# indutny/elliptic

Hardware: NVIDIA H100
Metric: secp256k1 ECDSA verifies/sec (higher is better)
Workload: dtype u32 limbs (integer, exact)

## Files before the change

elliptic_b200/csrc/eb200.cu:

```cuda
#include <cuda_runtime.h>
#include <stdio.h>
#include <string.h>
#include <atomic>
#include <condition_variable>
#include <cstdlib>
#include <mutex>
#include <thread>
#include <type_traits>
#include <vector>
#include "../../include/elliptic_b200.h"
#include "ecdsa_k256_body.cuh"
#include "ecdsa_k256_replay.cuh"
#include "ecdsa_sw_replay.cuh"
#include "ecdsa_k256_sign_fast.cuh"
#include "der_sig.cuh"
#include "ecdsa_sw_sign.cuh"
#include "ecdsa_k256_sign.cuh"
#include "ecdsa_sw_body.cuh"
#include "ed25519_body.cuh"
#include "ed25519_ec.cuh"
#include "sw_runtime.cuh"
#include "kernel_bounds.h"
#include "recovery_param.h"
#include "keyset.h"

using namespace eb;

__global__ void __launch_bounds__(128) k256_gtab_kernel(u32* gtab) {
  size_t t = (size_t)blockIdx.x * blockDim.x + threadIdx.x;
  if (t >= (size_t)GTAB_WINDOWS * GTAB_ENTRIES) return;
  int j = (int)(t / GTAB_ENTRIES), idx = (int)(t % GTAB_ENTRIES);
  gtab_entry(j, idx, gtab + t * 16);
}

__global__ void __launch_bounds__(128) k256_prep_kernel(size_t N, const uint8_t* __restrict__ e,
                                                        const uint8_t* __restrict__ r,
                                                        const uint8_t* __restrict__ s,
                                                        u32* __restrict__ ws, u32* __restrict__ scratch) {
  size_t tid = (size_t)blockIdx.x * blockDim.x + threadIdx.x;
  size_t T = (size_t)gridDim.x * blockDim.x;
  prep_thread(tid, T, N, e, r, s, ws, scratch);
}

__global__ void __launch_bounds__(EB_VERIFY_BLOCK, EB_VERIFY_MINBLOCKS)
k256_verify_kernel(size_t N, const uint8_t* __restrict__ pub, const uint8_t* __restrict__ r,
                   const u32* __restrict__ ws, const u32* __restrict__ gtab,
                   u32* __restrict__ qtab, const uint8_t* __restrict__ pre, uint8_t* __restrict__ status) {
  size_t i = (size_t)blockIdx.x * blockDim.x + threadIdx.x;
  if (i >= N) return;
  if (pre && pre[i]) { status[i] = pre[i]; return; }
  status[i] = verify_item(i, N, pub, r, ws, gtab, qtab);
}

__global__ void __launch_bounds__(128) k256_prep_recover_kernel(size_t N, const uint8_t* __restrict__ e,
                                                                const uint8_t* __restrict__ r,
                                                                const uint8_t* __restrict__ s,
                                                                u32* __restrict__ ws, u32* __restrict__ scratch) {
  size_t tid = (size_t)blockIdx.x * blockDim.x + threadIdx.x;
  size_t T = (size_t)gridDim.x * blockDim.x;
  prep_thread(tid, T, N, e, r, s, ws, scratch, 1);
}
__global__ void __launch_bounds__(EB_VERIFY_BLOCK, EB_VERIFY_MINBLOCKS)
k256_recover_kernel(size_t N, const uint8_t* __restrict__ r, const uint8_t* __restrict__ recid,
                    const u32* __restrict__ ws, const u32* __restrict__ gtab, u32* __restrict__ qtab,
                    uint8_t* __restrict__ out, uint8_t* __restrict__ status) {
  size_t i = (size_t)blockIdx.x * blockDim.x + threadIdx.x;
  if (i >= N) return;
  status[i] = recover_item(i, N, r, recid, ws, gtab, qtab, out);
}

__global__ void __launch_bounds__(128)
k256_sign_nonce_kernel(size_t N, const uint8_t* __restrict__ e, const uint8_t* __restrict__ priv,
                       const u32* __restrict__ gtab, u32* __restrict__ ws, uint8_t* __restrict__ status,
                       const uint8_t* __restrict__ kgiven) {
  size_t i = (size_t)blockIdx.x * blockDim.x + threadIdx.x;
  if (i < N) k256_sign_nonce_item(i, N, e, priv, gtab, ws, status, kgiven);
}
__global__ void __launch_bounds__(128)
k256_sign_finish_kernel(size_t N, const uint8_t* __restrict__ e, const uint8_t* __restrict__ priv, u32 canonical,
                        const u32* __restrict__ ws, u32* __restrict__ scratch, uint8_t* __restrict__ r,
                        uint8_t* __restrict__ s, uint8_t* __restrict__ recid, uint8_t* __restrict__ status) {
  size_t tid = (size_t)blockIdx.x * blockDim.x + threadIdx.x;
  size_t T = (size_t)gridDim.x * blockDim.x;
  k256_sign_finish_thread(tid, T, N, e, priv, canonical, ws, scratch, r, s, recid, status);
}
__global__ void __launch_bounds__(128)
k256_sign_slow_kernel(size_t N, const uint8_t* __restrict__ e, const uint8_t* __restrict__ priv, u32 canonical,
                      const u32* __restrict__ gtab, uint8_t* __restrict__ r, uint8_t* __restrict__ s,
                      uint8_t* __restrict__ recid, uint8_t* __restrict__ status) {
  size_t i = (size_t)blockIdx.x * blockDim.x + threadIdx.x;
  if (i >= N || status[i] != ST_NEEDS_HOST) return;
  status[i] = k256_sign_item(i, e, priv, canonical, gtab, r, s, recid);
}

__global__ void __launch_bounds__(128) k256_replay_tab_kernel(u32* tab) {
  int t = blockIdx.x * blockDim.x + threadIdx.x;
  if (t < 2 * REPLAY_NAF_PTS) rp_tab_entry(t, tab + 16 * t);
}
__global__ void __launch_bounds__(128)
k256_replay_kernel(size_t N, const uint8_t* __restrict__ e, const uint8_t* __restrict__ r, const uint8_t* __restrict__ s,
                   const uint8_t* __restrict__ pub, const u32* __restrict__ tab, uint8_t* __restrict__ status) {
  size_t i = (size_t)blockIdx.x * blockDim.x + threadIdx.x;
  if (i >= N || status[i] != ST_NEEDS_HOST) return;
  status[i] = rp_verify_item(i, e, r, s, pub, tab);
}

__global__ void __launch_bounds__(128)
k256_prep_scalars_kernel(size_t N, const uint8_t* __restrict__ k1, const uint8_t* __restrict__ k2, u32* __restrict__ ws) {
  size_t i = (size_t)blockIdx.x * blockDim.x + threadIdx.x;
  if (i < N) prep_scalars_item(i, N, k1, k2, ws);
}
__global__ void __launch_bounds__(EB_VERIFY_BLOCK, EB_VERIFY_MINBLOCKS)
k256_mul_add_kernel(size_t N, const uint8_t* __restrict__ pts, const u32* __restrict__ ws, const u32* __restrict__ gtab,
                    u32* __restrict__ qtab, uint8_t* __restrict__ out, uint8_t* __restrict__ status) {
  size_t i = (size_t)blockIdx.x * blockDim.x + threadIdx.x;
  if (i >= N) return;
  status[i] = mul_add_item(i, N, pts, ws, gtab, qtab, out);
}
__global__ void __launch_bounds__(128)
k256_mul_add_replay_kernel(size_t N, const uint8_t* __restrict__ k1, const uint8_t* __restrict__ k2,
                           const uint8_t* __restrict__ pts, const u32* __restrict__ tab, uint8_t* __restrict__ out,
                           uint8_t* __restrict__ status) {
  size_t i = (size_t)blockIdx.x * blockDim.x + threadIdx.x;
  if (i >= N || status[i] != ST_NEEDS_HOST) return;
  status[i] = rp_mul_add_item(i, k1, k2, pts, tab, out);
}
__global__ void __launch_bounds__(128)
// ... 398 lines not shown
    for (auto& t : workers_) t.join();
  }
 private:
  void loop() {
    unsigned long long seen = 0;
    for (;;) {
      { std::unique_lock<std::mutex> lk(m_); cv_work_.wait(lk, [&] { return stop_ || gen_ != seen; }); if (stop_) return; seen = gen_; }
      work();
    }
  }
  void work() {
    for (;;) {
      int i = next_.fetch_add(1);
      if (i >= njobs_.load()) break;
      const CopyJob* j = jobs_.load();
      memcpy(j[i].dst, j[i].src, j[i].bytes);
      std::lock_guard<std::mutex> lk(m_);
      if (--pending_ == 0) cv_done_.notify_all();
    }
  }
  std::mutex m_, call_mu_;
  std::condition_variable cv_work_, cv_done_;
  std::vector<std::thread> workers_;
  std::atomic<const CopyJob*> jobs_{nullptr};
  std::atomic<int> njobs_{0}, next_{0};
  int pending_ = 0;
  unsigned long long gen_ = 0;
  bool stop_ = false;
};

enum { EV_START, EV_INPUTS_RESIDENT, EV_KERNELS_DONE, EV_OUTPUTS_HOME, EV_MAIN_BEGIN, EV_MAIN_END, EV_SLOTS };

struct Ctx {
  std::mutex mu;
  bool ready = false;
  int device = -1;
  cudaStream_t stream = nullptr, stream2 = nullptr, copy_stream = nullptr;
  u32* gtab[MAX_CURVES] = {};
  u32* sw_replay_tab[MAX_CURVES] = {};
  u32* replay_tab = nullptr;
  uint8_t* d_in = nullptr; size_t d_in_cap = 0;
  uint8_t* d_ws = nullptr; size_t d_ws_cap = 0;
  uint8_t* d_status = nullptr; size_t d_status_cap = 0;
  cudaEvent_t ev[EV_SLOTS] = {};
  cudaEvent_t ev_in[MAX_CHUNKS] = {}, ev_k0[MAX_CHUNKS] = {}, ev_k1[MAX_CHUNKS] = {}, ev_done[MAX_CHUNKS] = {};
  uint8_t* h_stage[STAGE_SLOTS] = {};
  cudaEvent_t ev_stage[STAGE_SLOTS] = {};
  bool stage_used[STAGE_SLOTS] = {};
  unsigned stage_next = 0;
  CopyPool pool;
  eb200_timing timing = {};
};
Ctx g_ctx[MAX_DEV];
int g_devs[MAX_DEV];
int g_ndev = 0;
std::atomic<unsigned> g_rr{0};
std::mutex g_mu;
thread_local char g_err[256] = "";
thread_local eb200_timing t_timing = {};
thread_local Ctx* t_pending = nullptr;
thread_local unsigned t_pending_launches = 0;

int cuda_fail(cudaError_t e, const char* what) {
  snprintf(g_err, sizeof g_err, "%s: %s", what, cudaGetErrorString(e));
  return (e == cudaErrorNoDevice || e == cudaErrorInsufficientDriver) ? EB200_ERR_NO_DEVICE : EB200_ERR_CUDA;
}
#define CK(call) do { cudaError_t e_ = (call); if (e_ != cudaSuccess) return cuda_fail(e_, #call); } while (0)

struct Launch {
  cudaStream_t st;
  unsigned count = 0;
  int rc = EB200_OK;
  template <class... P, class... A>
  void operator()(void (*kernel)(P...), unsigned grid, unsigned block, A... args) {
    if (rc) return;
    kernel<<<grid, block, 0, st>>>(args...);
    count++;
    cudaError_t e = cudaGetLastError();
    if (e != cudaSuccess) rc = cuda_fail(e, "cudaGetLastError()");
  }
};
unsigned blocks128(size_t threads) { return (unsigned)((threads + 127) / 128); }
unsigned batch_blocks(size_t n, int batch) { return blocks128((n + batch - 1) / batch); }

struct K256Curve {};
struct Ed25519Curve {};
template <class C_> struct SwCurve {
  typedef C_ C;
  typedef SWSign<C, std::conditional_t<std::is_same<C, P384>::value, Sha384W,
                                       std::conditional_t<std::is_same<C, P521>::value, Sha512W, Sha256W>>> SG;
};
template <class T> constexpr bool is_k256 = std::is_same<T, K256Curve>::value;
template <class T> constexpr bool is_ed25519 = std::is_same<T, Ed25519Curve>::value;

template <class F>
int with_curve(int curve, F&& f) {
  switch (curve) {
    case EB200_CURVE_SECP256K1: return f(K256Curve{});
    case EB200_CURVE_ED25519: return f(Ed25519Curve{});
    case EB200_CURVE_P256: return f(SwCurve<P256>{});
    case EB200_CURVE_P384: return f(SwCurve<P384>{});
    case EB200_CURVE_P521: return f(SwCurve<P521>{});
    case EB200_CURVE_P192: return f(SwCurve<P192>{});
    case EB200_CURVE_P224: return f(SwCurve<P224>{});
    default: return EB200_ERR_UNSUPPORTED;
  }
}

[[maybe_unused]] const void* const sw_kernel_order[] = {
    (const void*)sw_decode_pub_kernel<P256>, (const void*)sw_decode_pub_kernel<P384>, (const void*)sw_decode_pub_kernel<P521>,
    (const void*)sw_decode_pub_kernel<P192>, (const void*)sw_decode_pub_kernel<P224>,
    (const void*)sw_keygen_kernel<SwCurve<P256>::SG>, (const void*)sw_keygen_kernel<SwCurve<P384>::SG>,
    (const void*)sw_keygen_kernel<SwCurve<P521>::SG>, (const void*)sw_keygen_kernel<SwCurve<P192>::SG>,
    (const void*)sw_keygen_kernel<SwCurve<P224>::SG>,
    (const void*)sw_mul_g_kernel<P256>, (const void*)sw_mul_g_kernel<P384>, (const void*)sw_mul_g_kernel<P521>,
    (const void*)sw_mul_g_kernel<P192>, (const void*)sw_mul_g_kernel<P224>,
    (const void*)sw_selftest_fe_kernel<P256>, (const void*)sw_selftest_fe_kernel<P384>, (const void*)sw_selftest_fe_kernel<P521>,
    (const void*)sw_selftest_fe_kernel<P192>, (const void*)sw_selftest_fe_kernel<P224>,
};

int grow(uint8_t** p, size_t* cap, size_t need) {
  if (*cap >= need) return EB200_OK;
  if (*p) { cudaFree(*p); *p = nullptr; *cap = 0; }
  CK(cudaMalloc(p, need));
  *cap = need;
  return EB200_OK;
}
size_t align256(size_t x) { return (x + 255) & ~(size_t)255; }

size_t fe_len(int curve) {
  if (curve == EB200_CURVE_P192) return 24;
  return (curve == EB200_CURVE_P384) ? 48 : (curve == EB200_CURVE_P521) ? 72 :
         ((curve >= EB200_CURVE_SECP256K1 && curve <= EB200_CURVE_CURVE25519) || curve == EB200_CURVE_P224) ? 32 : 0;
}
size_t curve_len(int curve) {
  switch (curve) {
    case EB200_CURVE_SECP256K1: case EB200_CURVE_P256: case EB200_CURVE_ED25519: return 32;
    case EB200_CURVE_P384: return 48;
    case EB200_CURVE_P521: return 66;
    case EB200_CURVE_P192: return 24;
    case EB200_CURVE_P224: return 28;
    default: return 0;
  }
}
size_t pub_item_bytes(size_t len, u32 fmt) {
  return fmt == EB200_PUB_XY ? 2 * len : fmt == EB200_PUB_SEC1_65 ? 1 + 2 * len : fmt == EB200_PUB_SEC1_33 ? 1 + len : 0;
}

struct WsLayout { size_t ws, scratch, qtab, xy, pre, total; };
WsLayout ws_layout(int curve, size_t n) {
  size_t prep_words = 0, scratch_words = 0, qtab_words = 0, len = curve_len(curve);
  with_curve(curve, [&](auto cv) {
    typedef decltype(cv) T;
    if constexpr (is_k256<T>) { prep_words = PREP_WORDS; scratch_words = 8; qtab_words = QTAB_WORDS; }
    else if constexpr (is_ed25519<T>) qtab_words = ED_ATAB_WORDS;
    else { typedef SW<typename T::C> W; prep_words = W::PREP_WORDS; scratch_words = W::N; qtab_words = W::QTAB_WORDS; }
    return EB200_OK;
  });
  WsLayout L;
  L.ws = 0;
  L.scratch = align256(L.ws + prep_words * n * 4);
  L.qtab = align256(L.scratch + scratch_words * n * 4);
  L.xy = align256(L.qtab + qtab_words * n * 4);
  L.pre = align256(L.xy + 2 * len * n);
  L.total = align256(L.pre + n);
  return L;
// ... 41 lines not shown
          CK(cudaMemcpyAsync(dsts[j], jobs[j].dst, jobs[j].bytes, cudaMemcpyHostToDevice, st));
          CK(cudaEventRecord(c.ev_stage[slots[j]], st));
          c.stage_used[slots[j]] = true;
        }
        nj = 0;
      }
    }
  }
  if (nj) {
    c.pool.run(jobs, nj);
    for (int j = 0; j < nj; j++) {
      CK(cudaMemcpyAsync(dsts[j], jobs[j].dst, jobs[j].bytes, cudaMemcpyHostToDevice, st));
      CK(cudaEventRecord(c.ev_stage[slots[j]], st));
      c.stage_used[slots[j]] = true;
    }
  }
  return EB200_OK;
}

int ensure_table(Ctx& c, int curve) {
  return with_curve(curve, [&](auto cv) {
    typedef decltype(cv) T;
    if (c.gtab[curve]) return EB200_OK;
    if constexpr (is_k256<T>) {
      size_t entries = (size_t)GTAB_WINDOWS * GTAB_ENTRIES;
      CK(cudaMalloc(&c.gtab[curve], entries * 16 * 4));
      k256_gtab_kernel<<<blocks128(entries), 128, 0, c.stream>>>(c.gtab[curve]);
      CK(cudaGetLastError());
      CK(cudaMalloc(&c.replay_tab, (size_t)REPLAY_TAB_WORDS * 4));
      k256_replay_tab_kernel<<<2, 128, 0, c.stream>>>(c.replay_tab);
    } else if constexpr (is_ed25519<T>) {
      size_t entries = (size_t)ED_GWINDOWS * ED_GENTRIES;
      CK(cudaMalloc(&c.gtab[curve], entries * 24 * 4));
      ed_gtab_kernel<<<blocks128(entries), 128, 0, c.stream>>>(c.gtab[curve]);
    } else {
      typedef typename T::C C;
      typedef SW<C> W;
      size_t entries = (size_t)W::GWINDOWS * W::GENTRIES;
      CK(cudaMalloc(&c.gtab[curve], entries * 2 * W::N * 4));
      sw_gtab_kernel<C><<<blocks128(entries), 128, 0, c.stream>>>(c.gtab[curve]);
      CK(cudaGetLastError());
      CK(cudaMalloc(&c.sw_replay_tab[curve], (size_t)SWReplay<C>::TAB_WORDS * 4));
      sw_replay_tab_kernel<C><<<1, 128, 0, c.stream>>>(c.sw_replay_tab[curve]);
    }
    CK(cudaGetLastError());
    CK(cudaStreamSynchronize(c.stream));
    return EB200_OK;
  });
}

int launch_verify(Ctx& c, int curve, size_t n, const uint8_t* d_e, const uint8_t* d_r, const uint8_t* d_s,
                  const uint8_t* d_pub, u32 pub_fmt, uint8_t* d_status, uint8_t* d_workspace, Launch& L,
                  cudaEvent_t ev_main0, cudaEvent_t ev_main1,
                  const uint8_t* d_der = nullptr, const unsigned long long* d_der_off = nullptr) {
  if (n == 0) return EB200_OK;
  const WsLayout W = ws_layout(curve, n);
  u32* ws = (u32*)(d_workspace + W.ws);
  u32* scratch = (u32*)(d_workspace + W.scratch);
  u32* qtab = (u32*)(d_workspace + W.qtab);
  uint8_t* dxy = d_workspace + W.xy;
  uint8_t* dpre = d_workspace + W.pre;
  const uint8_t* xy = d_pub;
  const uint8_t* pre = nullptr;
  const unsigned nb = blocks128(n);
  const u32* gt = c.gtab[curve];
  return with_curve(curve, [&](auto cv) {
    typedef decltype(cv) T;
    if (pub_fmt != EB200_PUB_XY) {
      if constexpr (is_k256<T>) L(k256_decode_pub_kernel, nb, 128, n, d_pub, pub_fmt, dxy, dpre);
      else if constexpr (is_ed25519<T>) L(ed_ec_decode_pub_kernel, nb, 128, n, d_pub, pub_fmt, dxy, dpre);
      else L(sw_decode_pub_kernel<typename T::C>, nb, 128, n, d_pub, pub_fmt, dxy, dpre);
      xy = dxy; pre = dpre;
    }
    if (d_der) {
      L(der_decode_kernel, nb, 128, n, (u32)curve_len(curve), d_der, d_der_off, (uint8_t*)d_r, (uint8_t*)d_s, dpre,
        (int)(pre != nullptr));
      pre = dpre;
    }
    if constexpr (is_ed25519<T>) {
      CK(cudaEventRecord(ev_main0, L.st));
      L(ed_ec_verify_kernel, nb, 128, n, d_e, d_r, d_s, xy, pre, gt, qtab, d_status);
      CK(cudaEventRecord(ev_main1, L.st));
    } else if constexpr (is_k256<T>) {
      L(k256_prep_kernel, batch_blocks(n, PREP_BATCH), 128, n, d_e, d_r, d_s, ws, scratch);
      CK(cudaEventRecord(ev_main0, L.st));
      L(k256_verify_kernel, (unsigned)((n + EB_VERIFY_BLOCK - 1) / EB_VERIFY_BLOCK), EB_VERIFY_BLOCK, n, xy, d_r, ws, gt,
        qtab, pre, d_status);
      CK(cudaEventRecord(ev_main1, L.st));
      L(k256_replay_kernel, nb, 128, n, d_e, d_r, d_s, xy, c.replay_tab, d_status);
    } else {
      typedef typename T::C C;
      L(sw_prep_kernel<C>, batch_blocks(n, SW<C>::BATCH), 128, n, d_e, d_r, d_s, ws, scratch);
      CK(cudaEventRecord(ev_main0, L.st));
      L(sw_verify_kernel<C>, nb, 128, n, xy, d_r, ws, gt, qtab, pre, d_status);
      CK(cudaEventRecord(ev_main1, L.st));
      L(sw_replay_kernel<C>, nb, 128, n, d_e, d_r, d_s, xy, c.sw_replay_tab[curve], d_status);
    }
    return L.rc;
  });
}

bool curve_ok(int curve) { return curve_len(curve) != 0; }
bool fmt_ok(u32 fmt) { return fmt == EB200_PUB_XY || fmt == EB200_PUB_SEC1_65 || fmt == EB200_PUB_SEC1_33; }

int ctx_create(Ctx& c, int device) {
  CK(cudaSetDevice(device));
  c.device = device;
  CK(cudaStreamCreateWithFlags(&c.stream, cudaStreamNonBlocking));
  CK(cudaStreamCreateWithFlags(&c.copy_stream, cudaStreamNonBlocking));
  CK(cudaStreamCreateWithFlags(&c.stream2, cudaStreamNonBlocking));
  for (int i = 0; i < EV_SLOTS; i++) CK(cudaEventCreate(&c.ev[i]));
  for (int i = 0; i < MAX_CHUNKS; i++) {
    CK(cudaEventCreate(&c.ev_in[i]));
    CK(cudaEventCreate(&c.ev_k0[i]));
    CK(cudaEventCreate(&c.ev_k1[i]));
    CK(cudaEventCreate(&c.ev_done[i]));
  }
  c.ready = true;
  return EB200_OK;
}
void ctx_destroy(Ctx& c) {
  if (c.device < 0) return;
  cudaSetDevice(c.device);
  if (c.stream) cudaStreamSynchronize(c.stream);
  for (int k = 0; k < MAX_CURVES; k++) if (c.gtab[k]) { cudaFree(c.gtab[k]); c.gtab[k] = nullptr; }
  for (int k = 0; k < MAX_CURVES; k++) if (c.sw_replay_tab[k]) { cudaFree(c.sw_replay_tab[k]); c.sw_replay_tab[k] = nullptr; }
  if (c.replay_tab) { cudaFree(c.replay_tab); c.replay_tab = nullptr; }
  if (c.d_in) { cudaMemset(c.d_in, 0, c.d_in_cap); cudaFree(c.d_in); } c.d_in = nullptr; c.d_in_cap = 0;
  if (c.d_ws) { cudaMemset(c.d_ws, 0, c.d_ws_cap); cudaFree(c.d_ws); } c.d_ws = nullptr; c.d_ws_cap = 0;
  cudaFree(c.d_status); c.d_status = nullptr; c.d_status_cap = 0;
  for (int i = 0; i < EV_SLOTS; i++) if (c.ev[i]) { cudaEventDestroy(c.ev[i]); c.ev[i] = nullptr; }
  for (int i = 0; i < MAX_CHUNKS; i++) {
    if (c.ev_in[i]) { cudaEventDestroy(c.ev_in[i]); c.ev_in[i] = nullptr; }
    if (c.ev_k0[i]) { cudaEventDestroy(c.ev_k0[i]); c.ev_k0[i] = nullptr; }
    if (c.ev_k1[i]) { cudaEventDestroy(c.ev_k1[i]); c.ev_k1[i] = nullptr; }
    if (c.ev_done[i]) { cudaEventDestroy(c.ev_done[i]); c.ev_done[i] = nullptr; }
  }
  for (int s = 0; s < STAGE_SLOTS; s++) {
    if (c.h_stage[s]) { memset(c.h_stage[s], 0, STAGE_BYTES); cudaFreeHost(c.h_stage[s]); c.h_stage[s] = nullptr; }
    if (c.ev_stage[s]) { cudaEventDestroy(c.ev_stage[s]); c.ev_stage[s] = nullptr; }
    c.stage_used[s] = false;
  }
  if (c.stream) { cudaStreamDestroy(c.stream); c.stream = nullptr; }
  if (c.copy_stream) { cudaStreamDestroy(c.copy_stream); c.copy_stream = nullptr; }
  if (c.stream2) { cudaStreamDestroy(c.stream2); c.stream2 = nullptr; }
  c.ready = false;
  c.device = -1;
}

Ctx* ctx_of(const void* dptr) {
  cudaPointerAttributes a;
  if (cudaPointerGetAttributes(&a, dptr) != cudaSuccess) { cudaGetLastError(); return nullptr; }
  if (a.type != cudaMemoryTypeDevice && a.type != cudaMemoryTypeManaged) return nullptr;
  if (a.device < 0 || a.device >= MAX_DEV || !g_ctx[a.device].ready) return nullptr;
  return &g_ctx[a.device];
}

void merge_timing(eb200_timing& a, const eb200_timing& b) {
  if (b.h2d_ms > a.h2d_ms) a.h2d_ms = b.h2d_ms;
  if (b.kernel_ms > a.kernel_ms) a.kernel_ms = b.kernel_ms;
  if (b.d2h_ms > a.d2h_ms) a.d2h_ms = b.d2h_ms;
  if (b.main_kernel_ms > a.main_kernel_ms) a.main_kernel_ms = b.main_kernel_ms;
  a.launches += b.launches;
}

template <class F>
int run_sharded_on(const int* devs, int nd, size_t n, F&& fn) {
// ... 1004 lines not shown
namespace {
std::mutex g_ks_mu;
std::vector<eb200_keyset*> g_keysets;

void keyset_free_device(eb200_keyset* ks) {
  for (int i = 0; i < ks->ndev; i++) {
    KeysetDev& d = ks->dev[ks->devs[i]];
    if (cudaSetDevice(ks->devs[i]) != cudaSuccess) { cudaGetLastError(); continue; }
    cudaFree(d.xy); cudaFree(d.kst); cudaFree(d.tab);
    d = KeysetDev{};
  }
  ks->ndev = 0;
  ks->live = false;
}

int keyset_build_on(Ctx& c, eb200_keyset* ks, const uint8_t* pub, uint8_t* key_status) {
  const int curve = ks->curve;
  const size_t m = ks->m, len = curve_len(curve), pb = pub_item_bytes(len, ks->fmt);
  const int windows = keyset_windows(curve, (int)ks->W);
  int rc = ensure_table(c, curve);
  if (rc) return rc;
  KeysetDev& d = ks->dev[c.device];
  d.W = (int)ks->W;
  CK(cudaMalloc(&d.xy, 2 * len * m));
  CK(cudaMalloc(&d.kst, m));
  CK(cudaMalloc(&d.tab, keyset_key_bytes(curve, (int)ks->W) * m));
  if ((rc = grow(&c.d_in, &c.d_in_cap, align256(m * pb) + m))) return rc;
  if ((rc = grow(&c.d_ws, &c.d_ws_cap, m * windows * 3 * keyset_geom(curve).limbs * 4))) return rc;
  uint8_t *d_pub = c.d_in, *d_pre = c.d_in + align256(m * pb);
  return run_single(c, {{d_pub, pub, m * pb}},
    [&](Launch& L) {
      const uint8_t* pre = nullptr;
      if (ks->fmt == EB200_PUB_XY) CK(cudaMemcpyAsync(d.xy, d_pub, 2 * len * m, cudaMemcpyDeviceToDevice, L.st));
      else {
        pre = d_pre;
        int rc2 = with_curve(curve, [&](auto cv) {
          typedef decltype(cv) T;
          if constexpr (is_k256<T>) L(k256_decode_pub_kernel, blocks128(m), 128, m, d_pub, ks->fmt, d.xy, d_pre);
          else if constexpr (is_ed25519<T>) return EB200_ERR_UNSUPPORTED;
          else L(sw_decode_pub_kernel<typename T::C>, blocks128(m), 128, m, d_pub, ks->fmt, d.xy, d_pre);
          return L.rc;
        });
        if (rc2) return rc2;
      }
      cudaError_t err = keyset_build_launch(curve, m, d, pre, (u32*)c.d_ws, L.st, &L.count);
      return err == cudaSuccess ? EB200_OK : cuda_fail(err, "keyset_build_launch");
    },
    {{key_status, d.kst, m}}, {}, true);
}

int verify_keyed_on(Ctx& c, const eb200_keyset* ks, size_t n, const uint8_t* e, const uint8_t* r, const uint8_t* s,
                    const u32* key_idx, uint8_t* status) {
  const int curve = ks->curve;
  const KeysetDev& d = ks->dev[c.device];
  if (!d.tab) return EB200_ERR_NOT_INIT;
  int rc = ensure_table(c, curve);
  if (rc) return rc;
  const size_t len = curve_len(curve);
  const ChunkPlan P = make_plan(n);
  const size_t idx_bytes = align256(n * 4);
  if ((rc = grow(&c.d_in, &c.d_in_cap, idx_bytes + align256(n * 3 * len) + 1024))) return rc;
  const WsLayout W = ws_layout(curve, P.max_m);
  const size_t ws_slot = W.qtab;
  if ((rc = grow(&c.d_ws, &c.d_ws_cap, (P.chunks > 1 ? 2 : 1) * ws_slot))) return rc;
  if ((rc = grow(&c.d_status, &c.d_status_cap, n))) return rc;
  u32* d_idx = (u32*)c.d_in;
  uint8_t *d_e = c.d_in + idx_bytes, *d_r = d_e + n * len, *d_s = d_r + n * len;
  return run_chunked(c, P,
    [&](size_t lo, size_t m, Seg* seg) {
      seg[0] = {d_e + lo * len, e + lo * len, m * len};
      seg[1] = {d_r + lo * len, r + lo * len, m * len};
      seg[2] = {d_s + lo * len, s + lo * len, m * len};
      seg[3] = {d_idx + lo, key_idx + lo, m * 4};
      return 4;
    },
    [&](size_t lo, size_t m, Launch& L, int slot, int k) {
      u32* ws = (u32*)(c.d_ws + (size_t)slot * ws_slot + W.ws);
      u32* scratch = (u32*)(c.d_ws + (size_t)slot * ws_slot + W.scratch);
      const u32* replay = nullptr;
      int rc2 = with_curve(curve, [&](auto cv) {
        typedef decltype(cv) T;
        if constexpr (is_ed25519<T>) return EB200_ERR_UNSUPPORTED;
        else if constexpr (is_k256<T>) {
          L(k256_prep_kernel, batch_blocks(m, PREP_BATCH), 128, m, d_e + lo * len, d_r + lo * len, d_s + lo * len, ws, scratch);
          replay = c.replay_tab;
        } else {
          typedef typename T::C C;
          L(sw_prep_kernel<C>, batch_blocks(m, SW<C>::BATCH), 128, m, d_e + lo * len, d_r + lo * len, d_s + lo * len, ws, scratch);
          replay = c.sw_replay_tab[curve];
        }
        return L.rc;
      });
      if (rc2) return rc2;
      const KeyedVerifyArgs a{d_e + lo * len, d_r + lo * len, d_s + lo * len, d_idx + lo, c.d_status + lo, ws, c.gtab[curve], replay};
      cudaError_t err = keyset_verify_launch(curve, m, d, a, L.st, c.ev_k0[k], c.ev_k1[k], &L.count);
      return err == cudaSuccess ? EB200_OK : cuda_fail(err, "keyset_verify_launch");
    },
    [&](size_t lo, size_t m, Seg* seg) {
      seg[0] = {status + lo, c.d_status + lo, m};
      return 1;
    });
}
}

static void keysets_release_all() {
  std::lock_guard<std::mutex> lk(g_ks_mu);
  for (eb200_keyset* ks : g_keysets) keyset_free_device(ks);
  g_keysets.clear();
}

extern "C" {

int eb200_keyset_create(int curve, size_t m, const uint8_t* pub, uint32_t pub_fmt, uint32_t table_bits,
                        uint8_t* key_status, eb200_keyset** out) {
  if (out) *out = nullptr;
  if (!out || !pub || !key_status || m == 0 || m > 0xffffffffull || !fmt_ok(pub_fmt)) return EB200_ERR_ARG;
  if (table_bits && (table_bits < EB200_KEYSET_MIN_BITS || table_bits > EB200_KEYSET_MAX_BITS)) return EB200_ERR_ARG;
  if (!keyset_geom(curve).limbs) return EB200_ERR_UNSUPPORTED;
  if (!table_bits && !(table_bits = keyset_choose_bits(curve, m, EB200_KEYSET_DEFAULT_BUDGET))) {
    snprintf(g_err, sizeof g_err, "the tables of %zu keys do not fit the default budget at any width: pass table_bits", m);
    return EB200_ERR_ARG;
  }
  int devs[MAX_DEV], nd;
  { std::lock_guard<std::mutex> lk(g_mu); nd = g_ndev; for (int i = 0; i < nd; i++) devs[i] = g_devs[i]; }
  if (nd == 0) return EB200_ERR_NOT_INIT;
  eb200_keyset* ks = new eb200_keyset;
  ks->curve = curve; ks->m = m; ks->W = table_bits; ks->fmt = pub_fmt;
  ks->device_bytes = 2 * curve_len(curve) * m + m + keyset_key_bytes(curve, (int)table_bits) * m;
  t_pending = nullptr;
  eb200_timing tm = {};
  int rc = EB200_OK;
  for (int i = 0; i < nd && !rc; i++) {
    Ctx& c = g_ctx[devs[i]];
    std::lock_guard<std::mutex> lk(c.mu);
    cudaError_t e = cudaSetDevice(c.device);
    if (e != cudaSuccess) { rc = cuda_fail(e, "cudaSetDevice"); break; }
    ks->devs[ks->ndev++] = c.device;
    c.timing = eb200_timing{};
    rc = keyset_build_on(c, ks, pub, key_status);
    merge_timing(tm, c.timing);
  }
  t_timing = tm;
  if (rc) {
    keyset_free_device(ks);
    delete ks;
    return rc;
  }
  ks->live = true;
  { std::lock_guard<std::mutex> lk(g_ks_mu); g_keysets.push_back(ks); }
  *out = ks;
  return EB200_OK;
}

int eb200_keyset_info(const eb200_keyset* ks, int* curve, size_t* m, uint32_t* table_bits, size_t* device_bytes) {
  if (!ks) return EB200_ERR_ARG;
  if (curve) *curve = ks->curve;
  if (m) *m = ks->m;
  if (table_bits) *table_bits = ks->W;
  if (device_bytes) *device_bytes = ks->device_bytes;
  return EB200_OK;
}

int eb200_keyset_destroy(eb200_keyset* ks) {
  if (!ks) return EB200_OK;
  {
    std::lock_guard<std::mutex> lk(g_ks_mu);
    for (size_t i = 0; i < g_keysets.size(); i++)
// ... 22 lines not shown
```

elliptic_b200/csrc/ecdsa_k256_body.cuh:

```cuda
#pragma once
#include "ge_k256.cuh"
#include "sc_k256.cuh"
#ifndef EB_K256_FQ
#define EB_K256_FQ 0
#endif
#include "gq_k256.cuh"

namespace eb {

enum : uint8_t {
  ST_FALSE = 0, ST_TRUE = 1, ST_THROW_INVALID_POINT = 2, ST_THROW_NOT_VALIDATED = 3,
  ST_NEEDS_HOST = 4, ST_THROW_ASSERT = 5, ST_THROW_POINT_FORMAT = 6, ST_INFINITY = 7, ST_THROW_SECOND_KEY = 8, ST_THROW_SIG_FORMAT = 9,
  ST_THROW_NO_RECOVERY = 11,
};

constexpr int PREP_WORDS = 19;
constexpr u32 FL_INVALID = 1, FL_NEGG = 2, FL_NEG1 = 4, FL_NEG2 = 8, FL_NOG = 16;
constexpr int PREP_BATCH = 16;
constexpr int QTAB_ENTRIES = 8;
#if EB_K256_FQ
constexpr int QTAB_WORDS = QTABQ_WORDS;
#else
constexpr int QTAB_WORDS = QTAB_ENTRIES * 24;
#endif
// ... 8 lines not shown
struct madd_out { ge_jac r; fe h; };

#if defined(__CUDACC__)
#define EB_FN __host__ __device__ __noinline__
#else
#define EB_FN
#endif

EB_FN ge_jac jac_dbl(ge_jac p) { return jac_dbl_inl(p); }
EB_FN ge_jac jac_madd(ge_jac a, ge_aff p) { return jac_madd_inl(a, p); }

EB_HD madd_out jac_madd_h(const ge_jac& a, const ge_aff& p) {
  madd_out o;
  fe z2 = fe_sqr(a.z);
  fe u2 = fe_mul(p.x, z2);
  fe s2 = fe_mul(fe_mul(p.y, z2), a.z);
  fe h = fe_sub(a.x, u2);
  fe rr = fe_sub(a.y, s2);
  fe h2 = fe_sqr(h);
  fe h3 = fe_mul(h2, h);
  fe v = fe_mul(a.x, h2);
  o.r.x = fe_sub(fe_sub(fe_add(fe_sqr(rr), h3), v), v);
  o.r.y = fe_sub(fe_mul(rr, fe_sub(v, o.r.x)), fe_mul(a.y, h3));
  o.r.z = fe_mul(a.z, h);
  o.h = h;
  return o;
}

EB_HD fe fe_beta() {
  fe b;
  const u32 v[8] = {0x719501eeu, 0xc1396c28u, 0x12f58995u, 0x9cf04975u, 0xac3434e9u, 0x6e64479eu, 0x657c0710u, 0x7ae96a2bu};
  for (int i = 0; i < 8; i++) b.v[i] = v[i];
  return b;
}

EB_HD ge_aff k256_G() {
  ge_aff g;
  const u32 x[8] = {0x16f81798u, 0x59f2815bu, 0x2dce28d9u, 0x029bfcdbu, 0xce870b07u, 0x55a06295u, 0xf9dcbbacu, 0x79be667eu};
  const u32 y[8] = {0xfb10d4b8u, 0x9c47d08fu, 0xa6855419u, 0xfd17b448u, 0x0e1108a8u, 0x5da4fbfcu, 0x26a3c465u, 0x483ada77u};
  for (int i = 0; i < 8; i++) { g.x.v[i] = x[i]; g.y.v[i] = y[i]; }
  return g;
}

EB_HD void gtab_entry(int j, int idx, u32* out16) {
  ge_jac b = jac_from_aff(k256_G());
  for (int k = 0; k < GTAB_W * j; k++) b = jac_dbl(b);
  ge_aff base = jac_to_aff(b);
  u32 s = 2 * idx + 1;
  ge_jac acc = jac_infinity();
  for (int k = GTAB_W - 1; k >= 0; k--) {
    acc = jac_dbl(acc);
    if ((s >> k) & 1) acc = jac_madd(acc, base);
  }
  ge_aff r = jac_to_aff(acc);
  r.x = fe_normalize(r.x);
  r.y = fe_normalize(r.y);
  for (int i = 0; i < 8; i++) { out16[i] = r.x.v[i]; out16[8 + i] = r.y.v[i]; }
}

EB_HD void prep_store(size_t i, size_t N, u32* u1, const u32* u2, u32 flags, u32* ws) {
  u32 nn[8];
  K256N::n(nn);
  if ((u1[0] & 1) == 0) {
    sub_n<8>(u1, nn, u1);
    flags |= FL_NEGG;
  }
  u32 m1[5], m2[5];
  bool n1, n2;
  glv_split_odd(u2, m1, &n1, m2, &n2);
  if (n1) flags |= FL_NEG1;
  if (n2) flags |= FL_NEG2;
  for (int w = 0; w < 8; w++) {
    u32 hi = (w < 7) ? u1[w + 1] : 0;
    ws[(size_t)w * N + i] = (u1[w] >> 1) | (hi << 31);
  }
  for (int w = 0; w < 5; w++) {
    ws[(size_t)(8 + w) * N + i] = m1[w];
    ws[(size_t)(13 + w) * N + i] = m2[w];
  }
  ws[(size_t)18 * N + i] = flags;
}

EB_HD void prep_thread(size_t tid, size_t T, size_t N, const uint8_t* e, const uint8_t* r,
                       const uint8_t* s, u32* ws, u32* scratch, int mode = 0) {
  u32 R2[8], one[8], nn[8];
  K256N::r2(R2); K256N::r1(one); K256N::n(nn);
  u32 prod[8];
  copy_n<8>(prod, one);
  u32 invalid_mask = 0;
  int cnt = 0;
  for (int j = 0; j < PREP_BATCH; j++) {
    size_t i = tid + (size_t)j * T;
    if (i >= N) break;
    cnt = j + 1;
    u32 sv[8], rv[8];
    load_be<8>(sv, s + 32 * i);
    load_be<8>(rv, r + 32 * i);
    bool ok = sc_in_range(sv) && sc_in_range(rv);
    u32 sm[8];
    if (mode == 1) {
      sc_mont_mul(sm, rv, R2);
      ok = !is_zero_n<8>(sm);
    } else {
      sc_mont_mul(sm, sv, R2);
      if (mode == 2) ok = !is_zero_n<8>(sm);
    }
    if (!ok) invalid_mask |= 1u << j;
    cmov_n<8>(sm, one, !ok);
    for (int w = 0; w < 8; w++) scratch[(size_t)w * N + i] = prod[w];
    u32 t[8];
    sc_mont_mul(t, prod, sm);
    copy_n<8>(prod, t);
  }
  if (cnt == 0) return;
  u32 inv[8];
  sc_mont_inv(inv, prod);
  for (int j = cnt - 1; j >= 0; j--) {
    size_t i = tid + (size_t)j * T;
    bool ok = !((invalid_mask >> j) & 1);
    u32 sv[8], rv[8], ev[8], sm[8], pre[8], sinv[8], t[8];
    load_be<8>(sv, s + 32 * i);
    load_be<8>(rv, r + 32 * i);
    sc_mont_mul(sm, mode == 1 ? rv : sv, R2);
    cmov_n<8>(sm, one, !ok);
    for (int w = 0; w < 8; w++) pre[w] = scratch[(size_t)w * N + i];
    sc_mont_mul(sinv, inv, pre);
    sc_mont_mul(t, inv, sm);
    copy_n<8>(inv, t);
    u32 flags = (ok || mode == 1) ? 0 : FL_INVALID;
    load_be<8>(ev, e + 32 * i);
    u32 u1[8], u2[8];
    if (mode == 1) {
      u32 zero8[8] = {0, 0, 0, 0, 0, 0, 0, 0};
      cmov_n<8>(sinv, zero8, !ok);
      sc_mont_mul(u1, ev, sinv);
      if (!is_zero_n<8>(u1)) sub_n<8>(u1, nn, u1);
      sc_mont_mul(u2, sv, sinv);
    } else {
      sc_mont_mul(u1, ev, sinv);
      sc_mont_mul(u2, rv, sinv);
    }
    prep_store(i, N, u1, u2, flags, ws);
  }
}

EB_HD void prep_scalars_item(size_t i, size_t N, const uint8_t* k1, const uint8_t* k2, u32* ws) {
  u32 nn[8], u1[8] = {0, 0, 0, 0, 0, 0, 0, 0}, u2[8];
  K256N::n(nn);
  u32 flags = 0;
  if (k1) {
    load_be<8>(u1, k1 + 32 * i);
    if (geq_n<8>(u1, nn)) sub_n<8>(u1, u1, nn);
  } else {
    flags |= FL_NOG;
  }
  load_be<8>(u2, k2 + 32 * i);
  if (geq_n<8>(u2, nn)) sub_n<8>(u2, u2, nn);
  prep_store(i, N, u1, u2, flags, ws);
}

EB_HD void store_fe(u32* dst, const fe& a) { for (int i = 0; i < 8; i++) dst[i] = a.v[i]; }
EB_HD fe load_fe(const u32* src) { fe a; for (int i = 0; i < 8; i++) a.v[i] = src[i]; return a; }

#if EB_K256_FQ
EB_HD ge_jac k256_dsm(size_t i, size_t N, const ge_aff& Q, u32 flags, const u32* ws, const u32* gtab, u32* qtab) {
  u32* tab = qtab + (size_t)i * QTAB_WORDS;
  fqk<1> zglobal;
  {
    gq_jac Qj; Qj.x = fqk_from_fe(Q.x); Qj.y = fqk_from_fe(Q.y); Qj.z = fqk_one();
    gq_jac D = gq_dbl(Qj);
    fqk<1> C2 = fq_sqr(D.z);
    fqk<1> C3 = fq_mul(C2, D.z);
    gq_jac P;
    P.x = fq_mul(Qj.x, C2);
    P.y = fq_mul(Qj.y, C3);
    P.z = fqk_one();
    fq_store12(tab + 0, P.x); fq_store12(tab + FQ_PAD, P.y);
    for (int k = 1; k < QTAB_ENTRIES; k++) {
      gq_madd_out o = gq_madd_h(P, D.x, D.y);
      P = o.r;
      u32* e = tab + QTABQ_ENTRY_WORDS * k;
      fq_store12(e, P.x); fq_store12(e + FQ_PAD, P.y);
      fq_store12(e + 2 * FQ_PAD, o.h);
    }
    zglobal = fq_mul(P.z, D.z);
    const fqk<1> beta = fqk_from_fe(fe_beta());
    fqk<1> zs = fqk_one();
    for (int k = QTAB_ENTRIES - 1; k >= 0; k--) {
      u32* e = tab + QTABQ_ENTRY_WORDS * k;
      fqk<1> X = fq_load12(e), Y = fq_load12(e + FQ_PAD);
      fqk<1> hk = fqk_one();
      if (k > 0) hk = fq_load12(e + 2 * FQ_PAD);
      if (k < QTAB_ENTRIES - 1) {
        fqk<1> zs2 = fq_sqr(zs);
        fqk<1> zs3 = fq_mul(zs2, zs);
        X = fq_mul(X, zs2);
        Y = fq_mul(Y, zs3);
        fq_store12(e, X); fq_store12(e + FQ_PAD, Y);
      }
      fq_store12(e + 2 * FQ_PAD, fq_mul(X, beta));
      zs = fq_mul(zs, hk);
    }
  }

  gq_jac acc;
  acc.x = fqk_one(); acc.y = fqk_one(); acc.z = fqk_zero();
  for (int w = 32; w >= 0; w--) {
    if (w != 32)
      for (int d = 0; d < 4; d++) acc = gq_dbl(acc);
    for (int h = 0; h < 2; h++) {
      u32 word = ws[(size_t)((h ? 13 : 8) + (w >> 3)) * N + i];
      u32 nib = (word >> (4 * (w & 7))) & 15;
      bool dneg = (w != 32) && (nib < 8);
      u32 idx = (w == 32) ? (nib & 7) : (dneg ? 7 - nib : nib - 8);
      bool neg = dneg != (((flags & (h ? FL_NEG2 : FL_NEG1)) != 0));
      const u32* e = tab + QTABQ_ENTRY_WORDS * idx;
      gq_aff P;
      P.x = fq_load12(e + (h ? 2 * FQ_PAD : 0));
      P.y = fq_cneg(fq_load12(e + FQ_PAD), neg);
      if (w == 32 && h == 0) acc = gq_from_aff(P);
      else acc = gq_madd(acc, P);
    }
  }
  acc.z = fq_mul(acc.z, zglobal);

  if (!(flags & FL_NOG)) {
    for (int j = 0; j < GTAB_WINDOWS; j++) {
      const int pos = GTAB_W * j;
      u32 lo = ws[(size_t)(pos >> 5) * N + i];
      u32 hi = ((pos >> 5) < 7) ? ws[(size_t)((pos >> 5) + 1) * N + i] : 0u;
      u64 both = ((u64)hi << 32) | lo;
      u32 chunk = (u32)(both >> (pos & 31)) & ((1u << GTAB_W) - 1);
      const u32 half = 1u << (GTAB_W - 1);
      bool dneg = (j != GTAB_WINDOWS - 1) && (chunk < half);
      u32 idx = (j == GTAB_WINDOWS - 1) ? (chunk & (half - 1)) : (dneg ? half - 1 - chunk : chunk - half);
      bool neg = dneg != ((flags & FL_NEGG) != 0);
      const u32* ent = gtab + ((size_t)j * GTAB_ENTRIES + idx) * 16;
      gq_aff P;
      P.x = fqk_from_fe(load_fe(ent));
      P.y = fq_cneg(fqk_from_fe(load_fe(ent + 8)), neg);
      acc = gq_madd(acc, P);
    }
  }
  return gq_to_jac(acc);
}
#else
EB_HD ge_jac k256_dsm(size_t i, size_t N, const ge_aff& Q, u32 flags, const u32* ws, const u32* gtab, u32* qtab) {
  u32* tab = qtab + (size_t)i * QTAB_WORDS;
  fe zglobal;
  {
    ge_jac D = jac_dbl(jac_from_aff(Q));
    fe C2 = fe_sqr(D.z);
    fe C3 = fe_mul(C2, D.z);
    ge_aff Dp; Dp.x = D.x; Dp.y = D.y;
    ge_jac P;
    P.x = fe_mul(Q.x, C2);
    P.y = fe_mul(Q.y, C3);
    P.z = fe_one();
    store_fe(tab + 0, P.x); store_fe(tab + 8, P.y);
    for (int k = 1; k < QTAB_ENTRIES; k++) {
      madd_out o = jac_madd_h(P, Dp);
      P = o.r;
      store_fe(tab + 24 * k, P.x); store_fe(tab + 24 * k + 8, P.y);
      store_fe(tab + 24 * k + 16, o.h);
    }
    zglobal = fe_mul(P.z, D.z);
    fe beta = fe_beta();
    fe zs = fe_one();
    for (int k = QTAB_ENTRIES - 1; k >= 0; k--) {
      fe X = load_fe(tab + 24 * k), Y = load_fe(tab + 24 * k + 8);
      fe hk = fe_one();
      if (k > 0) hk = load_fe(tab + 24 * k + 16);
      if (k < QTAB_ENTRIES - 1) {
        fe zs2 = fe_sqr(zs);
        fe zs3 = fe_mul(zs2, zs);
        X = fe_mul(X, zs2);
        Y = fe_mul(Y, zs3);
        store_fe(tab + 24 * k, X); store_fe(tab + 24 * k + 8, Y);
      }
      store_fe(tab + 24 * k + 16, fe_mul(X, beta));
      zs = fe_mul(zs, hk);
    }
  }

  ge_jac acc = jac_infinity();
  for (int w = 32; w >= 0; w--) {
    if (w != 32)
      for (int d = 0; d < 4; d++) acc = jac_dbl(acc);
    for (int h = 0; h < 2; h++) {
      u32 word = ws[(size_t)((h ? 13 : 8) + (w >> 3)) * N + i];
      u32 nib = (word >> (4 * (w & 7))) & 15;
      bool dneg = (w != 32) && (nib < 8);
      u32 idx = (w == 32) ? (nib & 7) : (dneg ? 7 - nib : nib - 8);
      bool neg = dneg != (((flags & (h ? FL_NEG2 : FL_NEG1)) != 0));
      ge_aff P;
      P.x = load_fe(tab + 24 * idx + (h ? 16 : 0));
      P.y = load_fe(tab + 24 * idx + 8);
      P = aff_neg_if(P, neg);
      if (w == 32 && h == 0) acc = jac_from_aff(P);
      else acc = jac_madd(acc, P);
    }
  }
  acc.z = fe_mul(acc.z, zglobal);

  if (flags & FL_NOG) return acc;
  for (int j = 0; j < GTAB_WINDOWS; j++) {
    const int pos = GTAB_W * j;
    u32 lo = ws[(size_t)(pos >> 5) * N + i];
    u32 hi = ((pos >> 5) < 7) ? ws[(size_t)((pos >> 5) + 1) * N + i] : 0u;
    u64 both = ((u64)hi << 32) | lo;
    u32 chunk = (u32)(both >> (pos & 31)) & ((1u << GTAB_W) - 1);
    const u32 half = 1u << (GTAB_W - 1);
    bool dneg = (j != GTAB_WINDOWS - 1) && (chunk < half);
    u32 idx = (j == GTAB_WINDOWS - 1) ? (chunk & (half - 1)) : (dneg ? half - 1 - chunk : chunk - half);
    bool neg = dneg != ((flags & FL_NEGG) != 0);
    const u32* ent = gtab + ((size_t)j * GTAB_ENTRIES + idx) * 16;
    ge_aff P;
    P.x = load_fe(ent);
    P.y = load_fe(ent + 8);
    acc = jac_madd(acc, aff_neg_if(P, neg));
  }
  return acc;
}

#endif

EB_HD uint8_t verify_item(size_t i, size_t N, const uint8_t* pub, const uint8_t* r,
                          const u32* ws, const u32* gtab, u32* qtab) {
  u32 flags = ws[(size_t)18 * N + i];
  if (flags & FL_INVALID) return ST_FALSE;
  ge_aff Q;
  Q.x = fe_from_be(pub + 64 * i);
  Q.y = fe_from_be(pub + 64 * i + 32);
  if (!aff_on_curve(Q)) return ST_NEEDS_HOST;
  ge_jac acc = k256_dsm(i, N, Q, flags, ws, gtab, qtab);

  if (fe_is_zero(acc.z)) return ST_FALSE;
  fe z2 = fe_sqr(acc.z);
  fe rf = fe_from_be(r + 32 * i);
  if (fe_eq(acc.x, fe_mul(rf, z2))) return ST_TRUE;
  const u32 pmn[8] = {0x2fc9baeeu, 0x402da172u, 0x50b75fc4u, 0x45512319u, 0x00000001u, 0, 0, 0};
  if (!geq_n<8>(rf.v, pmn)) {
    u32 nn[8]; K256N::n(nn);
    fe rn;
    add_n<8>(rn.v, rf.v, nn);
    if (fe_eq(acc.x, fe_mul(rn, z2))) return ST_TRUE;
  }
  return ST_FALSE;
}

EB_HD uint8_t recover_item(size_t i, size_t N, const uint8_t* r, const uint8_t* recid,
                           const u32* ws, const u32* gtab, u32* qtab, uint8_t* out) {
  for (int b = 0; b < 64; b++) out[64 * i + b] = 0;
  u32 j = recid[i];
  bool odd = j & 1, second = (j >> 1) & 1;
  u32 rv[8];
  load_be<8>(rv, r + 32 * i);
  const u32 pmn[8] = {0x2fc9baeeu, 0x402da172u, 0x50b75fc4u, 0x45512319u, 0x00000001u, 0, 0, 0};
  if (second && geq_n<8>(rv, pmn)) return ST_THROW_SECOND_KEY;
  fe x; copy_n<8>(x.v, rv);
  if (second) { u32 nn[8]; K256N::n(nn); add_n<8>(x.v, rv, nn); }
  fe seven = fe_zero(); seven.v[0] = 7;
  fe y2 = fe_add(fe_mul(fe_sqr(x), x), seven);
  fe y = fe_sqrt_candidate(y2);
  if (!fe_eq(fe_sqr(y), y2)) return ST_THROW_INVALID_POINT;
  if (fe_is_odd(y) != odd) y = fe_neg(y);
// ... 61 lines not shown
```

elliptic_b200/csrc/kernel_bounds.h:

```cpp
#pragma once

#ifndef EB_VERIFY_BLOCK
#define EB_VERIFY_BLOCK 128
#endif
#ifndef EB_VERIFY_MINBLOCKS
#define EB_VERIFY_MINBLOCKS 3
#endif
#ifndef EB_SW_MINBLOCKS_BIG
#define EB_SW_MINBLOCKS_BIG 2
#endif
#ifndef EB_SW_MINBLOCKS8
#define EB_SW_MINBLOCKS8 4
#endif
```

Measured before the change: 42.20 million.

## Specialize k256 Q-table build, enlarge prep batch for large inputs, raise min blocks

Replaces the generic doubling-plus-mixed-add Q-table construction with a hand-inlined co-Z style build. It derives the doubled point directly from affine Q and computes the global Z as zs*2y, avoiding some field multiplications. For inputs of 2^20 items or more, the prep kernel now batches 32 inversions per thread, using a 64-bit invalid mask, to amortize more Montgomery inversions. The k256 verify kernel also gets its own min-blocks bound of 4, which raises occupancy but risks register spills.

```diff
diff --git a/elliptic_b200/csrc/eb200.cu b/elliptic_b200/csrc/eb200.cu
--- a/elliptic_b200/csrc/eb200.cu
+++ b/elliptic_b200/csrc/eb200.cu
@@ -36,13 +36,13 @@
 __global__ void __launch_bounds__(128) k256_prep_kernel(size_t N, const uint8_t* __restrict__ e,
                                                         const uint8_t* __restrict__ r,
                                                         const uint8_t* __restrict__ s,
-                                                        u32* __restrict__ ws, u32* __restrict__ scratch) {
+                                                        u32* __restrict__ ws, u32* __restrict__ scratch, int batch) {
   size_t tid = (size_t)blockIdx.x * blockDim.x + threadIdx.x;
   size_t T = (size_t)gridDim.x * blockDim.x;
-  prep_thread(tid, T, N, e, r, s, ws, scratch);
-}
-
-__global__ void __launch_bounds__(EB_VERIFY_BLOCK, EB_VERIFY_MINBLOCKS)
+  prep_thread(tid, T, N, e, r, s, ws, scratch, 0, batch);
+}
+
+__global__ void __launch_bounds__(EB_VERIFY_BLOCK, EB_K256_VERIFY_MINBLOCKS)
 k256_verify_kernel(size_t N, const uint8_t* __restrict__ pub, const uint8_t* __restrict__ r,
                    const u32* __restrict__ ws, const u32* __restrict__ gtab,
                    u32* __restrict__ qtab, const uint8_t* __restrict__ pre, uint8_t* __restrict__ status) {
@@ -607,6 +607,7 @@
 };
 unsigned blocks128(size_t threads) { return (unsigned)((threads + 127) / 128); }
 unsigned batch_blocks(size_t n, int batch) { return blocks128((n + batch - 1) / batch); }
+int k256_prep_batch(size_t n) { return n >= ((size_t)1 << 20) ? 32 : PREP_BATCH; }
 
 struct K256Curve {};
 struct Ed25519Curve {};
@@ -814,7 +815,7 @@
       L(ed_ec_verify_kernel, nb, 128, n, d_e, d_r, d_s, xy, pre, gt, qtab, d_status);
       CK(cudaEventRecord(ev_main1, L.st));
     } else if constexpr (is_k256<T>) {
-      L(k256_prep_kernel, batch_blocks(n, PREP_BATCH), 128, n, d_e, d_r, d_s, ws, scratch);
+      L(k256_prep_kernel, batch_blocks(n, k256_prep_batch(n)), 128, n, d_e, d_r, d_s, ws, scratch, k256_prep_batch(n));
       CK(cudaEventRecord(ev_main0, L.st));
       L(k256_verify_kernel, (unsigned)((n + EB_VERIFY_BLOCK - 1) / EB_VERIFY_BLOCK), EB_VERIFY_BLOCK, n, xy, d_r, ws, gt,
         qtab, pre, d_status);
@@ -1985,7 +1986,8 @@
         typedef decltype(cv) T;
         if constexpr (is_ed25519<T>) return EB200_ERR_UNSUPPORTED;
         else if constexpr (is_k256<T>) {
-          L(k256_prep_kernel, batch_blocks(m, PREP_BATCH), 128, m, d_e + lo * len, d_r + lo * len, d_s + lo * len, ws, scratch);
+          L(k256_prep_kernel, batch_blocks(m, k256_prep_batch(m)), 128, m, d_e + lo * len, d_r + lo * len, d_s + lo * len, ws,
+            scratch, k256_prep_batch(m));
           replay = c.replay_tab;
         } else {
           typedef typename T::C C;
diff --git a/elliptic_b200/csrc/ecdsa_k256_body.cuh b/elliptic_b200/csrc/ecdsa_k256_body.cuh
--- a/elliptic_b200/csrc/ecdsa_k256_body.cuh
+++ b/elliptic_b200/csrc/ecdsa_k256_body.cuh
@@ -114,14 +114,14 @@
 }
 
 EB_HD void prep_thread(size_t tid, size_t T, size_t N, const uint8_t* e, const uint8_t* r,
-                       const uint8_t* s, u32* ws, u32* scratch, int mode = 0) {
+                       const uint8_t* s, u32* ws, u32* scratch, int mode = 0, int batch = PREP_BATCH) {
   u32 R2[8], one[8], nn[8];
   K256N::r2(R2); K256N::r1(one); K256N::n(nn);
   u32 prod[8];
   copy_n<8>(prod, one);
-  u32 invalid_mask = 0;
+  u64 invalid_mask = 0;
   int cnt = 0;
-  for (int j = 0; j < PREP_BATCH; j++) {
+  for (int j = 0; j < batch; j++) {
     size_t i = tid + (size_t)j * T;
     if (i >= N) break;
     cnt = j + 1;
@@ -137,7 +137,7 @@
       sc_mont_mul(sm, sv, R2);
       if (mode == 2) ok = !is_zero_n<8>(sm);
     }
-    if (!ok) invalid_mask |= 1u << j;
+    if (!ok) invalid_mask |= (u64)1 << j;
     cmov_n<8>(sm, one, !ok);
     for (int w = 0; w < 8; w++) scratch[(size_t)w * N + i] = prod[w];
     u32 t[8];
@@ -277,43 +277,49 @@
   return gq_to_jac(acc);
 }
 #else
+EB_HD fe qtab_build(const ge_aff& Q, u32* tab) {
+  fe B = fe_sqr(Q.x);
+  fe E = fe_sqr(Q.y);
+  fe L = fe_sqr(E);
+  fe S = fe_dbl(fe_sub(fe_sub(fe_sqr(fe_add(Q.x, E)), B), L));
+  fe M = fe_add(B, fe_dbl(B));
+  fe L8 = fe_dbl(fe_dbl(fe_dbl(L)));
+  fe Dx = fe_sub(fe_sqr(M), fe_dbl(S));
+  fe Dy = fe_sub(fe_mul(M, fe_sub(S, Dx)), L8);
+  fe Px = S, Py = L8;
+  store_fe(tab + 0, Px); store_fe(tab + 8, Py);
+  for (int k = 1; k < QTAB_ENTRIES; k++) {
+    fe h = fe_sub(Px, Dx);
+    fe C = fe_sqr(h);
+    fe W1 = fe_mul(Px, C), W2 = fe_mul(Dx, C);
+    fe A2 = fe_mul(Dy, fe_sub(W1, W2));
+    fe dy = fe_sub(Py, Dy);
+    Px = fe_sub(fe_sub(fe_sqr(dy), W1), W2);
+    Py = fe_sub(fe_mul(dy, fe_sub(W2, Px)), A2);
+    Dx = W2; Dy = A2;
+    store_fe(tab + 24 * k, Px); store_fe(tab + 24 * k + 8, Py);
+    store_fe(tab + 24 * k + 16, h);
+  }
+  fe beta = fe_beta();
+  fe zs = fe_one();
+  for (int k = QTAB_ENTRIES - 1; k >= 0; k--) {
+    fe X = load_fe(tab + 24 * k), Y = load_fe(tab + 24 * k + 8);
+    if (k < QTAB_ENTRIES - 1) {
+      fe zs2 = fe_sqr(zs);
+      fe zs3 = fe_mul(zs2, zs);
+      X = fe_mul(X, zs2);
+      Y = fe_mul(Y, zs3);
+      store_fe(tab + 24 * k, X); store_fe(tab + 24 * k + 8, Y);
+    }
+    if (k > 0) zs = fe_mul(zs, load_fe(tab + 24 * k + 16));
+    store_fe(tab + 24 * k + 16, fe_mul(X, beta));
+  }
+  return fe_mul(zs, fe_dbl(Q.y));
+}
+
 EB_HD ge_jac k256_dsm(size_t i, size_t N, const ge_aff& Q, u32 flags, const u32* ws, const u32* gtab, u32* qtab) {
   u32* tab = qtab + (size_t)i * QTAB_WORDS;
-  fe zglobal;
-  {
-    ge_jac D = jac_dbl(jac_from_aff(Q));
-    fe C2 = fe_sqr(D.z);
-    fe C3 = fe_mul(C2, D.z);
-    ge_aff Dp; Dp.x = D.x; Dp.y = D.y;
-    ge_jac P;
-    P.x = fe_mul(Q.x, C2);
-    P.y = fe_mul(Q.y, C3);
-    P.z = fe_one();
-    store_fe(tab + 0, P.x); store_fe(tab + 8, P.y);
-    for (int k = 1; k < QTAB_ENTRIES; k++) {
-      madd_out o = jac_madd_h(P, Dp);
-      P = o.r;
-      store_fe(tab + 24 * k, P.x); store_fe(tab + 24 * k + 8, P.y);
-      store_fe(tab + 24 * k + 16, o.h);
-    }
-    zglobal = fe_mul(P.z, D.z);
-    fe beta = fe_beta();
-    fe zs = fe_one();
-    for (int k = QTAB_ENTRIES - 1; k >= 0; k--) {
-      fe X = load_fe(tab + 24 * k), Y = load_fe(tab + 24 * k + 8);
-      fe hk = fe_one();
-      if (k > 0) hk = load_fe(tab + 24 * k + 16);
-      if (k < QTAB_ENTRIES - 1) {
-        fe zs2 = fe_sqr(zs);
-        fe zs3 = fe_mul(zs2, zs);
-        X = fe_mul(X, zs2);
-        Y = fe_mul(Y, zs3);
-        store_fe(tab + 24 * k, X); store_fe(tab + 24 * k + 8, Y);
-      }
-      store_fe(tab + 24 * k + 16, fe_mul(X, beta));
-      zs = fe_mul(zs, hk);
-    }
-  }
+  fe zglobal = qtab_build(Q, tab);
 
   ge_jac acc = jac_infinity();
   for (int w = 32; w >= 0; w--) {
diff --git a/elliptic_b200/csrc/kernel_bounds.h b/elliptic_b200/csrc/kernel_bounds.h
--- a/elliptic_b200/csrc/kernel_bounds.h
+++ b/elliptic_b200/csrc/kernel_bounds.h
@@ -6,6 +6,9 @@
 #ifndef EB_VERIFY_MINBLOCKS
 #define EB_VERIFY_MINBLOCKS 3
 #endif
+#ifndef EB_K256_VERIFY_MINBLOCKS
+#define EB_K256_VERIFY_MINBLOCKS 4
+#endif
 #ifndef EB_SW_MINBLOCKS_BIG
 #define EB_SW_MINBLOCKS_BIG 2
 #endif
```

Measured after the change: 45.34 million, median of 6. +7.4%, better.
